# nv-tlabs/GEN3C

Hardware: NVIDIA H100
Metric: denoise-steps/sec, 7B DiT, 121-frame 720p latent (higher is better)
Workload: dtype bf16

## Files before the change

### gen3c_b200/_lib.py

```python
from __future__ import annotations

import ctypes as C
import os
from pathlib import Path

_HERE = Path(__file__).resolve().parent
LIB_PATH = _HERE / "lib" / "libgen3c_b200.so"


class G3CError(RuntimeError):
    pass


class DitConfig(C.Structure):
    _fields_ = [
        ("model_channels", C.c_int),
        ("num_blocks", C.c_int),
        ("num_heads", C.c_int),
        ("ffn_dim", C.c_int),
        ("context_dim", C.c_int),
        ("adaln_lora_dim", C.c_int),
        ("in_channels", C.c_int),
        ("out_channels", C.c_int),
        ("concat_padding_mask", C.c_int),
        ("max_frames", C.c_int),
        ("max_h", C.c_int),
        ("max_w", C.c_int),
        ("rope_h_ratio", C.c_float),
        ("rope_w_ratio", C.c_float),
        ("rope_t_ratio", C.c_float),
        ("base_fps", C.c_int),
    ]


class StepArgs(C.Structure):
    _fields_ = [
        ("xt", C.c_void_p),
        ("gt_latent", C.c_void_p),
        ("aug_noise", C.c_void_p),
        ("indicator", C.c_void_p),
        ("cond_mask", C.c_void_p),
        ("pose_cond", C.c_void_p),
        ("padding_mask", C.c_void_p),
        ("ctx_cond", C.c_void_p),
        ("ctx_uncond", C.c_void_p),
        ("sigma", C.c_float),
        ("sigma_next", C.c_float),
        ("sigma_data", C.c_float),
        ("sigma_aug", C.c_float),
        ("guidance", C.c_float),
        ("xt_next", C.c_void_p),
        ("cond_mask_uncond", C.c_void_p),
        ("net_output", C.c_void_p),
    ]


_P = C.c_void_p
_I = C.c_int
_F = C.c_float

SIGNATURES = {
    "g3c_last_error": (C.c_char_p, []),
    "g3c_version": (_I, []),
    "g3c_device_info": (_I, [C.POINTER(_I), C.POINTER(_I), C.POINTER(_I)]),
    "g3c_render_create": (_I, [_I, _I, _I, C.POINTER(_P)]),
    "g3c_render_destroy": (_I, [_P]),
    "g3c_render_set_deterministic": (_I, [_P, _I]),
    "g3c_forward_warp": (_I, [_P, _P, _P, _P, _P, _P, _I, _I, _I, _P, _P, _P, _P, _P]),
    "g3c_render_cache": (_I, [_P, _P, _P, _P, _P, _P, _I, _I, _I, _I, _I, _P, _P, _P, _P]),
    "g3c_bilinear_splatting": (_I, [_P, _P, _P, _P, _P, _I, _I, _I, _P, _P, _P]),
    "g3c_splat_indices": (_I, [_P, _I, _I, _I, _P, _P]),
    "g3c_unproject_points": (_I, [_P, _P, _P, _P, _I, _I, _I, _I, _P, _P]),
    "g3c_reliable_depth_mask": (_I, [_P, _I, _I, _I, _I, _F, _F, _P, _P]),
    "g3c_align_depth_nonrigid": (_I, [_P, _P, _P, _P, _P, _I, _I, _I, _F, _F, _P, _P]),
    "g3c_foreground_occlusion": (_I, [_P, _P, _P, _P, _I, _I, _I, _I, _P, _P, _P, _P]),
    "g3c_render_cache_occlusion": (_I, [_P, _P, _P, _P, _I, _I, _I, _I, _P, _P, _P, _I, _I, _P]),
    "g3c_gemm_bf16": (_I, [_P, _P, _P, _I, _I, _I, _I, _I, _I, _I, _P, _I, _P]),
    "g3c_gemm_norm_rope_bf16": (_I, [_P, _P, _P, _I, _I, _I, _I, _I, _I, _P, _P, _F, _P]),
    "g3c_attn_fwd": (_I, [_P, _P, _P, _P, _I, _I, _I, _I, _I, _I, _I, _F, _P]),
    "g3c_attn_fwd_sbhd": (_I, [_P, _P, _P, _P, _I, _I, _I, _I, _I, _I, _I, _I, _F, _P]),
    "g3c_attn_set_trace": (_I, [_P]),
    "g3c_ln_modulate": (_I, [_P, _P, _P, _P, _P, _I, _I, _F, _P]),
    "g3c_rmsnorm_rope": (_I, [_P, _I, _I, _I, _P, _P, _F, _P]),
    "g3c_dit_create": (_I, [C.POINTER(DitConfig), C.POINTER(_P)]),
    "g3c_dit_destroy": (_I, [_P]),
    "g3c_dit_load": (_I, [_P, C.c_char_p, _P, C.POINTER(C.c_int64), _I, _I]),
    "g3c_nccl_unique_id": (_I, [_P]),
    "g3c_dit_enable_cp": (_I, [_P, _P, _I, _I]),
    "g3c_dit_cp_export": (_I, [_P, _P]),
    "g3c_dit_cp_import": (_I, [_P, _P, _I]),
    "g3c_dit_cp_mode": (_I, [_P]),
    "g3c_dit_disable_cp": (_I, [_P]),
    "g3c_dit_enable_cfg_parallel": (_I, [_P, _I]),
    "g3c_dit_cfg_export": (_I, [_P, _P]),
    "g3c_dit_cfg_import": (_I, [_P, _P]),
    "g3c_dit_set_shape": (_I, [_P, _I, _I, _I, _I, _F]),
    "g3c_dit_forward": (_I, [_P, _P, _P, _P, _P, _F, _P, _P, _P]),
    "g3c_denoise_step": (_I, [_P, C.POINTER(StepArgs), _P]),
    "g3c_dit_profile": (_I, [_P, _I]),
    "g3c_dit_profile_read": (_I, [_P, C.POINTER(_F), C.POINTER(_I), _I]),
    "g3c_dit_profile_wait_ms": (_I, [_P, C.POINTER(_F)]),
    "g3c_dit_workspace_bytes": (C.c_int64, [_P]),
    "g3c_dit_last_launch_count": (_I, [_P]),
}

_lib = None


def load() -> C.CDLL:
    global _lib
    if _lib is not None:
        return _lib
    path = os.environ.get("GEN3C_B200_LIB", str(LIB_PATH))
    if not os.path.exists(path):
        raise G3CError(
            f"{path} not found: build it with `python -c 'import __graft_entry__ as g; g.build()'` "
            "(there is no CPU fallback)"
        )
    lib = C.CDLL(path)
    for name, (res, args) in SIGNATURES.items():
        fn = getattr(lib, name)
        fn.restype = res
        fn.argtypes = args
    _lib = lib
    return lib


def check(rc: int, what: str = "") -> None:
    if rc != 0:
        msg = load().g3c_last_error().decode("utf-8", "replace")
        raise G3CError(f"{what} failed with status {rc}: {msg}")


def ptr(t) -> int | None:
    if t is None:
        return None
    if not t.is_contiguous():
        raise G3CError("tensor passed to the C ABI must be contiguous")
    return t.data_ptr()


def stream_ptr() -> int:
    import torch

    return torch.cuda.current_stream().cuda_stream
```

### gen3c_b200/csrc/common.cuh

```cuda
#pragma once
#include <cuda.h>
#include <cuda_bf16.h>
#include <cuda_runtime.h>
#include <stdint.h>
#include <stdio.h>

#include "../../include/gen3c_b200.h"
#include "wgmma_ops.cuh"

namespace g3c {

void set_error(const char* fmt, ...);
int cuda_fail(cudaError_t e, const char* what, const char* file, int line);
#define G3C_CUDA(x)                                                         \
  do {                                                                      \
    cudaError_t _e = (x);                                                   \
    if (_e != cudaSuccess) return ::g3c::cuda_fail(_e, #x, __FILE__, __LINE__); \
  } while (0)
#define G3C_REQUIRE(cond, ...)        \
  do {                                \
    if (!(cond)) {                    \
      ::g3c::set_error(__VA_ARGS__);  \
      return G3C_EINVAL;       \
    }                                 \
  } while (0)

int make_tmap_bf16_sw128(CUtensorMap* out, const void* base, int rank, const uint64_t* dims,
                         const uint64_t* strides_bytes, const uint32_t* box);
int make_tmap_f32_sw128(CUtensorMap* out, const void* base, const uint64_t* dims,
                        const uint64_t* strides_bytes, const uint32_t* box);

int sm_count();

#ifdef __CUDACC__
__device__ __forceinline__ uint32_t smem_u32(const void* p) {
  return static_cast<uint32_t>(__cvta_generic_to_shared(p));
}
__device__ __forceinline__ uint32_t lane_id() { return threadIdx.x & 31; }
__device__ __forceinline__ uint32_t warp_id() { return __shfl_sync(0xffffffffu, threadIdx.x >> 5, 0); }

__device__ __forceinline__ bool elect_one() {
  uint32_t pred = 0;
  asm volatile(
      "{\n\t.reg .pred P;\n\t"
      "elect.sync _|P, 0xffffffff;\n\t"
      "selp.b32 %0, 1, 0, P;\n\t}\n"
      : "=r"(pred));
  return pred != 0;
}

__device__ __forceinline__ void mbar_init(uint64_t* bar, uint32_t count) {
  asm volatile("mbarrier.init.shared::cta.b64 [%0], %1;\n" ::"r"(smem_u32(bar)), "r"(count));
}
__device__ __forceinline__ void fence_barrier_init() {
  asm volatile("fence.mbarrier_init.release.cluster;\n" ::: "memory");
}
__device__ __forceinline__ void fence_proxy_async() {
  asm volatile("fence.proxy.async.shared::cta;\n" ::: "memory");
}
__device__ __forceinline__ void mbar_expect_tx(uint64_t* bar, uint32_t bytes) {
  asm volatile("mbarrier.arrive.expect_tx.shared::cta.b64 _, [%0], %1;\n" ::"r"(smem_u32(bar)),
               "r"(bytes)
               : "memory");
}
__device__ __forceinline__ void mbar_arrive(uint64_t* bar) {
  asm volatile("mbarrier.arrive.shared::cta.b64 _, [%0];\n" ::"r"(smem_u32(bar)) : "memory");
}
#ifndef G3C_MBAR_SUSPEND_NS
#define G3C_MBAR_SUSPEND_NS 0
#endif
__device__ __forceinline__ bool mbar_try_wait(uint64_t* bar, uint32_t parity) {
  uint32_t ok;
#if G3C_MBAR_SUSPEND_NS > 0
  asm volatile(
      "{\n\t.reg .pred P;\n\t"
      "mbarrier.try_wait.parity.shared::cta.b64 P, [%1], %2, %3;\n\t"
      "selp.b32 %0, 1, 0, P;\n\t}\n"
      : "=r"(ok)
      : "r"(smem_u32(bar)), "r"(parity), "r"((uint32_t)G3C_MBAR_SUSPEND_NS)
      : "memory");
#else
  asm volatile(
      "{\n\t.reg .pred P;\n\t"
      "mbarrier.try_wait.parity.shared::cta.b64 P, [%1], %2;\n\t"
      "selp.b32 %0, 1, 0, P;\n\t}\n"
      : "=r"(ok)
      : "r"(smem_u32(bar)), "r"(parity)
      : "memory");
#endif
  return ok != 0;
}
__device__ __forceinline__ bool mbar_test(uint64_t* bar, uint32_t parity) {
  uint32_t ok;
  asm volatile(
      "{\n\t.reg .pred P;\n\t"
      "mbarrier.test_wait.parity.shared::cta.b64 P, [%1], %2;\n\t"
      "selp.b32 %0, 1, 0, P;\n\t}\n"
      : "=r"(ok)
      : "r"(smem_u32(bar)), "r"(parity)
      : "memory");
  return ok != 0;
}
#ifndef G3C_MBAR_TIMEOUT_NS
#define G3C_MBAR_TIMEOUT_NS 4000000000ull
#endif
__device__ __forceinline__ uint64_t global_timer_ns() {
  uint64_t t;
  asm volatile("mov.u64 %0, %%globaltimer;\n" : "=l"(t));
  return t;
}
#ifdef G3C_MBAR_DEBUG
#define G3C_MBAR_TIMEOUT_ACTION(bar, parity)                                                                 \
  do {                                                                                                       \
    printf("g3c: mbarrier timeout block(%d,%d) thread %d bar@%u parity %u\n", blockIdx.x, blockIdx.y,        \
           threadIdx.x, bar, parity);                                                                        \
    __trap();                                                                                                \
  } while (0)
#else
#define G3C_MBAR_TIMEOUT_ACTION(bar, parity) asm volatile("trap;\n")
#endif
__device__ __forceinline__ void mbar_wait(uint64_t* bar, uint32_t parity) {
  if (mbar_try_wait(bar, parity)) return;
  uint32_t spins = 0;
  uint64_t t0 = 0;
  while (!mbar_try_wait(bar, parity)) {
    if ((++spins & 0xFFFu) == 0) {
      uint64_t now = global_timer_ns();
      if (t0 == 0) t0 = now;
      else if (now - t0 > G3C_MBAR_TIMEOUT_NS) G3C_MBAR_TIMEOUT_ACTION(smem_u32(bar), parity);
    }
  }
}

__device__ __forceinline__ void mbar_wait_ns(uint64_t* bar, uint32_t parity, unsigned long long timeout_ns) {
  if (mbar_try_wait(bar, parity)) return;
  uint32_t spins = 0;
  uint64_t t0 = 0;
  while (!mbar_try_wait(bar, parity)) {
    if ((++spins & 0xFFFu) == 0) {
      uint64_t now = global_timer_ns();
      if (t0 == 0) t0 = now;
      else if (now - t0 > timeout_ns) G3C_MBAR_TIMEOUT_ACTION(smem_u32(bar), parity);
    }
  }
}

__device__ __forceinline__ void mbar_wait_ns_or_exit(uint64_t* bar, uint32_t parity, unsigned long long timeout_ns) {
  if (mbar_try_wait(bar, parity)) return;
  uint32_t spins = 0;
  uint64_t t0 = 0;
  while (!mbar_try_wait(bar, parity)) {
    if ((++spins & 0xFFFu) == 0) {
      uint64_t now = global_timer_ns();
      if (t0 == 0) t0 = now;
      else if (now - t0 > timeout_ns) asm volatile("exit;\n");
    }
  }
}

__device__ __forceinline__ void tma_prefetch_desc(const CUtensorMap* m) {
  asm volatile("prefetch.tensormap [%0];\n" ::"l"(reinterpret_cast<uint64_t>(m)) : "memory");
}
__device__ __forceinline__ void tma_load_2d(void* smem_dst, const CUtensorMap* m, uint64_t* bar,
                                            int c0, int c1) {
  asm volatile(
      "cp.async.bulk.tensor.2d.shared::cluster.global.mbarrier::complete_tx::bytes"
      " [%0], [%1, {%3, %4}], [%2];\n" ::"r"(smem_u32(smem_dst)),
      "l"(reinterpret_cast<uint64_t>(m)), "r"(smem_u32(bar)), "r"(c0), "r"(c1)
      : "memory");
}
__device__ __forceinline__ void tma_load_3d(void* smem_dst, const CUtensorMap* m, uint64_t* bar,
                                            int c0, int c1, int c2) {
  asm volatile(
      "cp.async.bulk.tensor.3d.shared::cluster.global.mbarrier::complete_tx::bytes"
      " [%0], [%1, {%3, %4, %5}], [%2];\n" ::"r"(smem_u32(smem_dst)),
      "l"(reinterpret_cast<uint64_t>(m)), "r"(smem_u32(bar)), "r"(c0), "r"(c1), "r"(c2)
      : "memory");
}

__device__ __forceinline__ void tma_store_2d(const CUtensorMap* m, const void* smem_src, int c0, int c1) {
  asm volatile("cp.async.bulk.tensor.2d.global.shared::cta.bulk_group [%0, {%2, %3}], [%1];\n" ::"l"(
                   reinterpret_cast<uint64_t>(m)),
               "r"(smem_u32(smem_src)), "r"(c0), "r"(c1)
               : "memory");
}
__device__ __forceinline__ void tma_reduce_add_2d(const CUtensorMap* m, const void* smem_src, int c0, int c1) {
  asm volatile("cp.reduce.async.bulk.tensor.2d.global.shared::cta.add.bulk_group [%0, {%2, %3}], [%1];\n" ::"l"(
                   reinterpret_cast<uint64_t>(m)),
               "r"(smem_u32(smem_src)), "r"(c0), "r"(c1)
               : "memory");
}
__device__ __forceinline__ void tma_store_commit() { asm volatile("cp.async.bulk.commit_group;\n" ::: "memory"); }
template <int N>
__device__ __forceinline__ void tma_store_wait_read() {
  asm volatile("cp.async.bulk.wait_group.read %0;\n" ::"n"(N) : "memory");
}
template <int N>
__device__ __forceinline__ void tma_store_wait_all() {
  asm volatile("cp.async.bulk.wait_group %0;\n" ::"n"(N) : "memory");
}

__device__ __forceinline__ void wgmma_fence() { asm volatile("wgmma.fence.sync.aligned;\n" ::: "memory"); }
__device__ __forceinline__ void wgmma_commit() { asm volatile("wgmma.commit_group.sync.aligned;\n" ::: "memory"); }
template <int N>
__device__ __forceinline__ void wgmma_wait() {
  asm volatile("wgmma.wait_group.sync.aligned %0;\n" ::"n"(N) : "memory");
}
template <int N>
__device__ __forceinline__ void fence_regs(float (&r)[N]) {
#pragma unroll
  for (int i = 0; i < N; ++i) asm volatile("" : "+f"(r[i])::"memory");
}
template <int N>
__device__ __forceinline__ void fence_regs(uint32_t (&r)[N]) {
#pragma unroll
  for (int i = 0; i < N; ++i) asm volatile("" : "+r"(r[i])::"memory");
}

__device__ __forceinline__ uint64_t make_sdesc_sw128(uint32_t smem_addr) {
  uint64_t d = 0;
  d |= static_cast<uint64_t>((smem_addr & 0x3FFFFu) >> 4);
  d |= static_cast<uint64_t>(1) << 16;
  d |= static_cast<uint64_t>(1024u >> 4) << 32;
  d |= static_cast<uint64_t>(1) << 62;
  return d;
}
__device__ __forceinline__ uint64_t make_sdesc_sw128_mn(uint32_t smem_addr, uint32_t mn_block_bytes) {
  uint64_t d = 0;
  d |= static_cast<uint64_t>((smem_addr & 0x3FFFFu) >> 4);
  d |= static_cast<uint64_t>((mn_block_bytes >> 4) & 0x3FFFu) << 16;
  d |= static_cast<uint64_t>(1024u >> 4) << 32;
  d |= static_cast<uint64_t>(1) << 62;
  return d;
}
__device__ __forceinline__ uint64_t sdesc_advance(uint64_t d, uint32_t bytes) {
  return d + static_cast<uint64_t>(bytes >> 4);
}

template <int N>
__device__ __forceinline__ void setmaxnreg_dec() {
  asm volatile("setmaxnreg.dec.sync.aligned.u32 %0;\n" ::"n"(N));
}
template <int N>
__device__ __forceinline__ void setmaxnreg_inc() {
  asm volatile("setmaxnreg.inc.sync.aligned.u32 %0;\n" ::"n"(N));
}

__device__ __forceinline__ uint32_t pack_bf16x2(float lo, float hi) {
  __nv_bfloat162 v = __floats2bfloat162_rn(lo, hi);
  return *reinterpret_cast<uint32_t*>(&v);
}
__device__ __forceinline__ float warp_max(float v) {
#pragma unroll
  for (int o = 16; o > 0; o >>= 1) v = fmaxf(v, __shfl_xor_sync(0xffffffffu, v, o));
  return v;
}
__device__ __forceinline__ float warp_sum(float v) {
#pragma unroll
  for (int o = 16; o > 0; o >>= 1) v += __shfl_xor_sync(0xffffffffu, v, o);
  return v;
}
#endif

}
```

### gen3c_b200/csrc/gemm_wgmma.cu

```cuda
#include <cstdlib>
#include <cstring>

#include "kernels.h"

namespace g3c {

constexpr int BM = 128;
constexpr int BK = 64;
constexpr int WG_K = 16;
constexpr int GEMM_THREADS = 384;

struct GemmParams {
  int M, N, K;
  int ldd;
  void* D;
  const float* gate;
  int num_m_blk, num_n_blk, num_k_blk;
  int super_n;
  const float* nr_gamma;
  const float* nr_cs;
  float nr_eps;
};

constexpr int EPI_NORM_ROPE_BF16 = 4;

template <int BN>
struct GemmSmem {
  static constexpr int kABytes = BM * BK * 2;
  static constexpr int kBBytes = BN * BK * 2;
  static constexpr int kStageBytes = kABytes + kBBytes;
  static constexpr int kStages = (192 * 1024) / kStageBytes;
  static constexpr int kBarBytes = 256;
  static constexpr int kTotal = kStages * kStageBytes + kBarBytes + 1024;
};

__device__ __forceinline__ float gelu_erf(float x) {
  return 0.5f * x * (1.0f + erff(x * 0.70710678118654752440f));
}

__device__ __forceinline__ void tile_coords(const GemmParams& p, int tile, int& m_blk, int& n_blk) {
  int per_super = p.num_m_blk * p.super_n;
  int sc = tile / per_super;
  int rem = tile - sc * per_super;
  int n0 = sc * p.super_n;
  int width = p.num_n_blk - n0 < p.super_n ? p.num_n_blk - n0 : p.super_n;
  m_blk = rem / width;
  n_blk = n0 + rem - m_blk * width;
}

template <int BN>
__device__ __forceinline__ void epilogue_norm_rope(const float (&acc)[BN / 2], const GemmParams& p, int row_a, int col_q,
                                                   int n_base) {
#pragma unroll
  for (int hd = 0; hd < BN / 128; ++hd) {
    if (n_base + hd * 128 >= p.N) break;
    float ss[2] = {0.f, 0.f};
#pragma unroll
    for (int i = 16 * hd; i < 16 * hd + 16; ++i) {
      ss[0] = fmaf(acc[4 * i], acc[4 * i], fmaf(acc[4 * i + 1], acc[4 * i + 1], ss[0]));
      ss[1] = fmaf(acc[4 * i + 2], acc[4 * i + 2], fmaf(acc[4 * i + 3], acc[4 * i + 3], ss[1]));
    }
#pragma unroll
    for (int h = 0; h < 2; ++h) {
      ss[h] += __shfl_xor_sync(0xffffffffu, ss[h], 1);
      ss[h] += __shfl_xor_sync(0xffffffffu, ss[h], 2);
    }
#pragma unroll
    for (int h = 0; h < 2; ++h) {
      const int row = row_a + 8 * h;
      if (row >= p.M) continue;
      const float rstd = rsqrtf(ss[h] * (1.0f / 128.0f) + p.nr_eps);
      const float* cs = p.nr_cs ? p.nr_cs + (size_t)row * 128 : nullptr;
      __nv_bfloat16* dptr = reinterpret_cast<__nv_bfloat16*>(p.D) + (size_t)row * p.ldd + n_base + hd * 128;
#pragma unroll
      for (int i = 0; i < 8; ++i) {
        const int c = 8 * i + col_q;
        const float2 ga = *reinterpret_cast<const float2*>(p.nr_gamma + c);
        const float2 gb = *reinterpret_cast<const float2*>(p.nr_gamma + 64 + c);
        const int ia = 4 * (16 * hd + i) + 2 * h, ib = 4 * (16 * hd + i + 8) + 2 * h;
        float a[2] = {acc[ia] * (rstd * ga.x), acc[ia + 1] * (rstd * ga.y)};
        float b[2] = {acc[ib] * (rstd * gb.x), acc[ib + 1] * (rstd * gb.y)};
        if (cs) {
          const float2 co = *reinterpret_cast<const float2*>(cs + c);
          const float2 si = *reinterpret_cast<const float2*>(cs + 64 + c);
          const float cv[2] = {co.x, co.y}, sv[2] = {si.x, si.y};
#pragma unroll
          for (int e = 0; e < 2; ++e) {
            const float n = a[e] * cv[e] - b[e] * sv[e], m = b[e] * cv[e] + a[e] * sv[e];
            a[e] = n;
            b[e] = m;
          }
        }
        *reinterpret_cast<uint32_t*>(dptr + c) = pack_bf16x2(a[0], a[1]);
        *reinterpret_cast<uint32_t*>(dptr + 64 + c) = pack_bf16x2(b[0], b[1]);
      }
    }
  }
}

template <int BN, int EPI>
__device__ __forceinline__ void epilogue(const float (&acc)[BN / 2], const GemmParams& p, int row_a, int col_q,
                                         int n_base) {
  if constexpr (EPI == EPI_NORM_ROPE_BF16) {
    epilogue_norm_rope<BN>(acc, p, row_a, col_q, n_base);
  } else {
#pragma unroll
    for (int h = 0; h < 2; ++h) {
      const int row = row_a + 8 * h;
      if (row >= p.M) continue;
#pragma unroll
      for (int i = 0; i < BN / 8; ++i) {
        const int col = n_base + 8 * i + col_q;
        if (col >= p.N) continue;
        const bool pair = col + 1 < p.N;
        float v0 = acc[4 * i + 2 * h], v1 = acc[4 * i + 2 * h + 1];
        if constexpr (EPI == G3C_EPI_BF16 || EPI == G3C_EPI_GELU_BF16) {
          if constexpr (EPI == G3C_EPI_GELU_BF16) {
            v0 = gelu_erf(v0);
            v1 = gelu_erf(v1);
          }
          __nv_bfloat16* dptr = reinterpret_cast<__nv_bfloat16*>(p.D) + (size_t)row * p.ldd + col;
          if (pair) *reinterpret_cast<uint32_t*>(dptr) = pack_bf16x2(v0, v1);
          else dptr[0] = __float2bfloat16_rn(v0);
        } else {
          float* dptr = reinterpret_cast<float*>(p.D) + (size_t)row * p.ldd + col;
          if constexpr (EPI == G3C_EPI_GATED_RESIDUAL_F32) {
            if (pair) {
              const float2 g = *reinterpret_cast<const float2*>(p.gate + col);
              float2 x = *reinterpret_cast<float2*>(dptr);
              x.x = fmaf(g.x, v0, x.x);
              x.y = fmaf(g.y, v1, x.y);
              *reinterpret_cast<float2*>(dptr) = x;
            } else {
              dptr[0] = fmaf(p.gate[col], v0, dptr[0]);
            }
          } else {
            if (pair) *reinterpret_cast<float2*>(dptr) = make_float2(v0, v1);
            else dptr[0] = v0;
          }
        }
      }
    }
  }
}

template <int BN, int EPI>
__global__ void __launch_bounds__(GEMM_THREADS, 1)
    k_gemm(const __grid_constant__ CUtensorMap tmA, const __grid_constant__ CUtensorMap tmB, const GemmParams p) {
  using S = GemmSmem<BN>;
  constexpr int kStages = S::kStages;
  extern __shared__ uint8_t smem_raw[];
  uint8_t* smem = reinterpret_cast<uint8_t*>((reinterpret_cast<uintptr_t>(smem_raw) + 1023) &
                                             ~static_cast<uintptr_t>(1023));
  uint8_t* smem_a = smem;
  uint8_t* smem_b = smem + kStages * S::kABytes;
  uint64_t* bars = reinterpret_cast<uint64_t*>(smem + kStages * S::kStageBytes);
  uint64_t* full = bars;
  uint64_t* empty = bars + kStages;

  const uint32_t wg = threadIdx.x / 128;
  const uint32_t tid = threadIdx.x % 128;

  if (threadIdx.x == 0) {
    tma_prefetch_desc(&tmA);
    tma_prefetch_desc(&tmB);
    for (int i = 0; i < kStages; ++i) {
      mbar_init(&full[i], 1);
      mbar_init(&empty[i], 2);
    }
    fence_barrier_init();
  }
  __syncthreads();

  const int num_tiles = p.num_m_blk * p.num_n_blk;

  if (wg == 0) {
    setmaxnreg_dec<40>();
    if (tid == 0) {
      uint32_t stage = 0, phase = 0;
      for (int tile = blockIdx.x; tile < num_tiles; tile += gridDim.x) {
        int m_blk, n_blk;
        tile_coords(p, tile, m_blk, n_blk);
        for (int kb = 0; kb < p.num_k_blk; ++kb) {
          mbar_wait(&empty[stage], phase ^ 1);
          mbar_expect_tx(&full[stage], S::kStageBytes);
          tma_load_2d(smem_a + stage * S::kABytes, &tmA, &full[stage], kb * BK, m_blk * BM);
          tma_load_2d(smem_b + stage * S::kBBytes, &tmB, &full[stage], kb * BK, n_blk * BN);
          if (++stage == kStages) {
            stage = 0;
            phase ^= 1;
          }
        }
      }
    }
  } else {
    setmaxnreg_inc<232>();
    const uint32_t c = wg - 1;
    const uint32_t warp = tid / 32, lane = tid % 32;
    uint32_t stage = 0, phase = 0;
    float acc[BN / 2];
    for (int tile = blockIdx.x; tile < num_tiles; tile += gridDim.x) {
      int m_blk, n_blk;
      tile_coords(p, tile, m_blk, n_blk);
      uint32_t prev_stage = 0;
      for (int kb = 0; kb < p.num_k_blk; ++kb) {
        mbar_wait(&full[stage], phase);
        const uint64_t da = make_sdesc_sw128(smem_u32(smem_a + stage * S::kABytes + c * 64 * 128));
        const uint64_t db = make_sdesc_sw128(smem_u32(smem_b + stage * S::kBBytes));
        wgmma_fence();
#pragma unroll
        for (int k = 0; k < BK / WG_K; ++k) {
          const uint64_t a = sdesc_advance(da, k * WG_K * 2), b = sdesc_advance(db, k * WG_K * 2);
          const uint32_t accumulate = (kb | k) != 0 ? 1u : 0u;
          if constexpr (BN == 256) wgmma_ss_n256(acc, a, b, accumulate);
          else if constexpr (BN == 128) wgmma_ss_n128(acc, a, b, accumulate);
          else wgmma_ss_n64(acc, a, b, accumulate);
        }
        wgmma_commit();
        wgmma_wait<1>();
        fence_regs(acc);
        if (kb > 0 && tid == 0) mbar_arrive(&empty[prev_stage]);
        prev_stage = stage;
        if (++stage == kStages) {
          stage = 0;
          phase ^= 1;
        }
      }
      wgmma_wait<0>();
      fence_regs(acc);
      if (tid == 0) mbar_arrive(&empty[prev_stage]);
      epilogue<BN, EPI>(acc, p, m_blk * BM + (int)(c * 64 + warp * 16 + lane / 4), (int)(2 * (lane % 4)), n_blk * BN);
    }
  }
}

template <int BN, int EPI>
static int launch_gemm(const CUtensorMap& tmA, const CUtensorMap& tmB, const GemmParams& p, cudaStream_t st) {
  using S = GemmSmem<BN>;
  static bool configured = false;
  if (!configured) {
    G3C_CUDA(cudaFuncSetAttribute(k_gemm<BN, EPI>, cudaFuncAttributeMaxDynamicSharedMemorySize, S::kTotal));
    configured = true;
  }
  int tiles = p.num_m_blk * p.num_n_blk;
  int grid = tiles < sm_count() ? tiles : sm_count();
  k_gemm<BN, EPI><<<grid, GEMM_THREADS, S::kTotal, st>>>(tmA, tmB, p);
  G3C_CUDA(cudaGetLastError());
  return G3C_OK;
}

template <int BN>
static int dispatch_epi(int epi, const CUtensorMap& tmA, const CUtensorMap& tmB, const GemmParams& p, cudaStream_t st) {
  switch (epi) {
    case G3C_EPI_BF16: return launch_gemm<BN, G3C_EPI_BF16>(tmA, tmB, p, st);
    case G3C_EPI_GELU_BF16: return launch_gemm<BN, G3C_EPI_GELU_BF16>(tmA, tmB, p, st);
    case G3C_EPI_GATED_RESIDUAL_F32: return launch_gemm<BN, G3C_EPI_GATED_RESIDUAL_F32>(tmA, tmB, p, st);
    case G3C_EPI_F32: return launch_gemm<BN, G3C_EPI_F32>(tmA, tmB, p, st);
    case EPI_NORM_ROPE_BF16:
      if constexpr (BN >= 128) return launch_gemm<BN, EPI_NORM_ROPE_BF16>(tmA, tmB, p, st);
      break;
  }
  set_error("gemm: unknown epilogue %d", epi);
  return G3C_EINVAL;
}

int gemm_bf16(const void* A, const void* B, void* D, int M, int N, int K, int lda, int ldb, int ldd,
              int epilogue, const float* gate, int block_n, cudaStream_t st, const NormRope* norm_rope) {
  G3C_REQUIRE(A && B && D, "gemm: null operand");
  if (norm_rope) {
    G3C_REQUIRE(epilogue == G3C_EPI_BF16 && N % 128 == 0 && norm_rope->gamma,
                "gemm: the RMSNorm/RoPE epilogue needs the bf16 epilogue, N %% 128 == 0 and a gain vector");
    G3C_REQUIRE((reinterpret_cast<uintptr_t>(norm_rope->gamma) & 15) == 0 &&
                    (reinterpret_cast<uintptr_t>(norm_rope->cs) & 15) == 0,
                "gemm: RMSNorm gain / RoPE table must be 16-byte aligned");
    epilogue = EPI_NORM_ROPE_BF16;
  }
  G3C_REQUIRE(M > 0 && N > 0 && K > 0, "gemm: bad shape %dx%dx%d", M, N, K);
  G3C_REQUIRE(K % 8 == 0 && lda % 8 == 0 && ldb % 8 == 0, "gemm: K/lda/ldb must be multiples of 8");
  G3C_REQUIRE(lda >= K && ldb >= K && ldd >= N, "gemm: leading dimension smaller than extent");
  if (epilogue == G3C_EPI_BF16 || epilogue == G3C_EPI_GELU_BF16 || epilogue == EPI_NORM_ROPE_BF16)
    G3C_REQUIRE(ldd % 8 == 0 && (reinterpret_cast<uintptr_t>(D) & 15) == 0,
                "gemm: bf16 output needs ldd %% 8 == 0 and 16-byte aligned base");
  else
    G3C_REQUIRE(ldd % 4 == 0 && (reinterpret_cast<uintptr_t>(D) & 15) == 0,
                "gemm: f32 output needs ldd %% 4 == 0 and 16-byte aligned base");
  G3C_REQUIRE(epilogue != G3C_EPI_GATED_RESIDUAL_F32 ||
                  (gate && (reinterpret_cast<uintptr_t>(gate) & 15) == 0),
              "gemm: gated-residual epilogue needs a 16-byte aligned gate vector");
  int bn = block_n;
  G3C_REQUIRE(bn == 0 || bn == 64 || bn == 128 || bn == 256 || bn == 512, "gemm: block_n %d unsupported", bn);
  if (bn == 512) {
    G3C_REQUIRE(N % 256 == 0, "gemm: block_n 512 needs N %% 256 == 0 (N=%d)", N);
    bn = 256;
  }
  if (bn == 0) bn = (N >= 256 && N % 256 == 0) ? 256 : (N > 64 ? 128 : 64);
  G3C_REQUIRE(epilogue != EPI_NORM_ROPE_BF16 || bn >= 128, "gemm: the RMSNorm/RoPE epilogue needs tiles of whole heads");

  CUtensorMap tmA, tmB;
  uint64_t dimsA[2] = {(uint64_t)K, (uint64_t)M}, strA[1] = {(uint64_t)lda * 2};
  uint32_t boxA[2] = {BK, BM};
  int rc = make_tmap_bf16_sw128(&tmA, A, 2, dimsA, strA, boxA);
  if (rc) return rc;
  uint64_t dimsB[2] = {(uint64_t)K, (uint64_t)N}, strB[1] = {(uint64_t)ldb * 2};
  uint32_t boxB[2] = {BK, (uint32_t)bn};
  rc = make_tmap_bf16_sw128(&tmB, B, 2, dimsB, strB, boxB);
  if (rc) return rc;

  GemmParams p;
  p.M = M;
  p.N = N;
  p.K = K;
  p.ldd = ldd;
  p.D = D;
  p.gate = gate;
  p.nr_gamma = norm_rope ? norm_rope->gamma : nullptr;
  p.nr_cs = norm_rope ? norm_rope->cs : nullptr;
  p.nr_eps = norm_rope ? norm_rope->eps : 0.0f;
  p.num_m_blk = (M + BM - 1) / BM;
  p.num_n_blk = (N + bn - 1) / bn;
  p.num_k_blk = (K + BK - 1) / BK;
  long long col_bytes = (long long)bn * K * 2;
  int sn = (int)((16ll << 20) / (col_bytes > 0 ? col_bytes : 1));
  if (sn < 1) sn = 1;
  if (sn > p.num_n_blk) sn = p.num_n_blk;
  p.super_n = sn;
  switch (bn) {
    case 64: return dispatch_epi<64>(epilogue, tmA, tmB, p, st);
    case 128: return dispatch_epi<128>(epilogue, tmA, tmB, p, st);
    default: return dispatch_epi<256>(epilogue, tmA, tmB, p, st);
  }
}

}

extern "C" int g3c_gemm_bf16(const void* A, const void* B, void* D, int M, int N, int K, int lda,
                             int ldb, int ldd, int epilogue, const float* gate, int block_n,
                             void* stream) {
  return g3c::gemm_bf16(A, B, D, M, N, K, lda, ldb, ldd, epilogue, gate, block_n,
                        (cudaStream_t)stream);
}

extern "C" int g3c_gemm_norm_rope_bf16(const void* A, const void* B, void* D, int M, int N, int K, int lda, int ldb,
                                       int ldd, const float* gamma, const float* cos_sin, float eps, void* stream) {
  g3c::NormRope nr;
  nr.gamma = gamma;
  nr.cs = cos_sin;
  nr.eps = eps;
  return g3c::gemm_bf16(A, B, D, M, N, K, lda, ldb, ldd, G3C_EPI_BF16, nullptr, 0, (cudaStream_t)stream, &nr);
}
```

### gen3c_b200/ops.py

```python
from __future__ import annotations

from typing import Optional

import torch

from . import _lib

EPI_BF16, EPI_GELU_BF16, EPI_GATED_RESIDUAL_F32, EPI_F32 = 0, 1, 2, 3


def _chk(t: torch.Tensor, dtype, name: str):
    if not t.is_cuda or t.dtype != dtype or not t.is_contiguous():
        raise ValueError(f"{name} must be a contiguous CUDA tensor of dtype {dtype}")


def gemm(a: torch.Tensor, b: torch.Tensor, epilogue: int = EPI_BF16, out: Optional[torch.Tensor] = None,
         gate: Optional[torch.Tensor] = None, block_n: int = 0) -> torch.Tensor:
    _chk(a, torch.bfloat16, "a")
    _chk(b, torch.bfloat16, "b")
    M, K = a.shape
    N, K2 = b.shape
    assert K == K2, "inner dimensions differ"
    odt = torch.bfloat16 if epilogue in (EPI_BF16, EPI_GELU_BF16) else torch.float32
    if out is None:
        if epilogue == EPI_GATED_RESIDUAL_F32:
            raise ValueError("gated-residual epilogue accumulates into `out`")
        out = torch.empty((M, N), device=a.device, dtype=odt)
    _chk(out, odt, "out")
    if gate is not None:
        _chk(gate, torch.float32, "gate")
    lib = _lib.load()
    with torch.cuda.device(a.device):
        _lib.check(lib.g3c_gemm_bf16(_lib.ptr(a), _lib.ptr(b), _lib.ptr(out), M, N, K, K, K, N, epilogue,
                                     _lib.ptr(gate), block_n, _lib.stream_ptr()), "g3c_gemm_bf16")
    return out


def gemm_norm_rope(a: torch.Tensor, b: torch.Tensor, gamma: torch.Tensor, cos_sin: Optional[torch.Tensor] = None,
                   eps: float = 1e-6) -> torch.Tensor:
    _chk(a, torch.bfloat16, "a")
    _chk(b, torch.bfloat16, "b")
    _chk(gamma, torch.float32, "gamma")
    M, K = a.shape
    N = b.shape[0]
    assert b.shape[1] == K and N % 128 == 0 and gamma.numel() == 128
    if cos_sin is not None:
        _chk(cos_sin, torch.float32, "cos_sin")
        assert tuple(cos_sin.shape) == (M, 128)
    out = torch.empty((M, N), device=a.device, dtype=torch.bfloat16)
    lib = _lib.load()
    with torch.cuda.device(a.device):
        _lib.check(lib.g3c_gemm_norm_rope_bf16(_lib.ptr(a), _lib.ptr(b), _lib.ptr(out), M, N, K, K, K, N, _lib.ptr(gamma),
                                               _lib.ptr(cos_sin), eps, _lib.stream_ptr()), "g3c_gemm_norm_rope_bf16")
    return out


def attention(q: torch.Tensor, k: torch.Tensor, vt: torch.Tensor, heads: int, scale: Optional[float] = None,
              vt_chunk_len: int = 0) -> torch.Tensor:
    for t, n in ((q, "q"), (k, "k"), (vt, "vt")):
        _chk(t, torch.bfloat16, n)
    Lq, Dq = q.shape
    Lk = k.shape[0]
    assert Dq == heads * 128 and k.shape[1] == heads * 128
    o = torch.empty_like(q)
    if scale is None:
        scale = 128 ** -0.5
    lib = _lib.load()
    with torch.cuda.device(q.device):
        _lib.check(lib.g3c_attn_fwd(_lib.ptr(q), _lib.ptr(k), _lib.ptr(vt), _lib.ptr(o), Lq, Lk, heads, Dq, Dq, Dq,
                                    vt_chunk_len, scale, _lib.stream_ptr()), "g3c_attn_fwd")
    return o


def _token_stride(t: torch.Tensor, name: str) -> int:
    if not t.is_cuda or t.dtype != torch.bfloat16:
        raise ValueError(f"{name} must be a bf16 CUDA tensor, got {t.dtype} on {t.device}")
    if t.dim() != 4 or t.shape[0] < 1 or t[0].numel() == 0:
        raise ValueError(f"{name} must be a non-empty [s, b, h, d] tensor, got shape {tuple(t.shape)}")
    if not t[0].is_contiguous():
        raise ValueError(f"the (b, h, d) block of {name} must be contiguous, got strides {t.stride()}")
    row = t[0].numel()
    ld = t.stride(0) if t.shape[0] > 1 else row
    if ld < row or ld % 8 != 0:
        raise ValueError(f"the token stride of {name} ({ld}) must be a multiple of 8 and >= b*h*d = {row}")
    if t.data_ptr() % 16 != 0:
        raise ValueError(f"{name} must start on a 16-byte boundary")
    return ld


def attention_sbhd(q: torch.Tensor, k: torch.Tensor, v: torch.Tensor, scale: Optional[float] = None) -> torch.Tensor:
    if q.dim() == 4 and q.shape[-1] != 128:
        raise NotImplementedError(f"head_dim {q.shape[-1]}: only 128 is implemented")
    if q.dim() == 4 and k.dim() == 4 and k.shape[2] != q.shape[2]:
        raise NotImplementedError(f"{k.shape[2]} key heads for {q.shape[2]} query heads: GQA is not implemented")
    ldq, ldk, ldv = _token_stride(q, "q"), _token_stride(k, "k"), _token_stride(v, "v")
    if k.shape != v.shape or k.shape[1:] != q.shape[1:]:
        raise ValueError(f"q {tuple(q.shape)}, k {tuple(k.shape)} and v {tuple(v.shape)} must agree in (b, h, d) "
                         "and k, v in s")
    if not (q.device == k.device == v.device):
        raise ValueError("q, k and v must be on one device")
    sq, b, h, d = q.shape
    o = torch.empty((sq, b, h * d), device=q.device, dtype=torch.bfloat16)
    if scale is None:
        scale = 128 ** -0.5
    lib = _lib.load()
    with torch.cuda.device(q.device):
        _lib.check(lib.g3c_attn_fwd_sbhd(q.data_ptr(), k.data_ptr(), v.data_ptr(), o.data_ptr(), sq, k.shape[0], b, h,
                                         ldq, ldk, ldv, b * h * d, scale, _lib.stream_ptr()), "g3c_attn_fwd_sbhd")
    return o


def ln_modulate(x: torch.Tensor, shift: torch.Tensor, scale: torch.Tensor, pos: Optional[torch.Tensor] = None,
                eps: float = 1e-6) -> torch.Tensor:
    _chk(x, torch.float32, "x")
    L, D = x.shape
    y = torch.empty((L, D), device=x.device, dtype=torch.bfloat16)
    lib = _lib.load()
    with torch.cuda.device(x.device):
        _lib.check(lib.g3c_ln_modulate(_lib.ptr(x), _lib.ptr(pos), _lib.ptr(shift), _lib.ptr(scale), _lib.ptr(y), L, D,
                                       eps, _lib.stream_ptr()), "g3c_ln_modulate")
    return y


def rmsnorm_rope_(qk: torch.Tensor, heads: int, gamma: torch.Tensor, cos_sin: Optional[torch.Tensor] = None,
                  eps: float = 1e-6) -> torch.Tensor:
    _chk(qk, torch.bfloat16, "qk")
    _chk(gamma, torch.float32, "gamma")
    L, ld = qk.shape
    lib = _lib.load()
    with torch.cuda.device(qk.device):
        _lib.check(lib.g3c_rmsnorm_rope(_lib.ptr(qk), ld, L, heads, _lib.ptr(gamma), _lib.ptr(cos_sin), eps,
                                        _lib.stream_ptr()), "g3c_rmsnorm_rope")
    return qk
```

### include/gen3c_b200.h

```cpp
#ifndef GEN3C_B200_H_
#define GEN3C_B200_H_

#include <stdint.h>

#ifdef __cplusplus
extern "C" {
#endif

#define G3C_OK 0
#define G3C_EINVAL (-1)
#define G3C_ECUDA (-2)
#define G3C_ENOMEM (-3)
#define G3C_ESTATE (-4)
#define G3C_ENCCL (-5)

const char* g3c_last_error(void);
int g3c_version(void);
int g3c_device_info(int* sm_count, int* cc_major, int* cc_minor);


typedef struct g3c_render g3c_render_t;

int g3c_render_create(int H, int W, int max_items_per_pass, g3c_render_t** out);
int g3c_render_destroy(g3c_render_t* r);

int g3c_render_set_deterministic(g3c_render_t* r, int on);

#define G3C_WARP_RENDER_DEPTH 1
#define G3C_WARP_NOT_IMAGE 2

int g3c_forward_warp(g3c_render_t* r, const float* points, const float* image, const float* mask,
                     const float* w2c, const float* K, int b, int C, int flags, float* warped,
                     float* mask_out, float* depth_out, float* flow_out, void* stream);

int g3c_render_cache(g3c_render_t* r, const float* points, const float* images, const float* masks,
                     const float* w2cs, const float* Ks, int B, int F_target, int N, int src_frames,
                     int render_depth, float* pixels, float* masks_out, float* depth_out,
                     void* stream);

int g3c_bilinear_splatting(g3c_render_t* r, const float* frame, const float* mask,
                           const float* depth, const float* flow, int b, int C, int is_image,
                           float* out, float* mask_out, void* stream);

int g3c_splat_indices(const float* flow, int b, int H, int W, int32_t* idx, void* stream);

int g3c_unproject_points(const float* depth, const float* w2c, const float* K, const uint8_t* mask,
                         int b, int H, int W, int is_depth, float* points, void* stream);

int g3c_reliable_depth_mask(const float* depth, int b, int H, int W, int window, float ratio_thresh,
                            float eps, uint8_t* out, void* stream);

int g3c_align_depth_nonrigid(const float* depth, const float* target_depth, const uint8_t* target_mask, const float* K,
                             const float* c2w, int H, int W, int num_iters, float lambda_arap, float lr,
                             float* out_depth, void* stream);

int g3c_foreground_occlusion(const float* points, const unsigned char* boundary, const float* w2c, const float* K, int b,
                             int C, int H, int W, float* warped, float* mask, float* depth, void* stream);

int g3c_render_cache_occlusion(const float* points, const unsigned char* boundary, const float* w2cs, const float* Ks, int B,
                               int F_target, int N, int src_frames, float* pixels, float* masks, float* depth, int H, int W,
                               void* stream);


#define G3C_EPI_BF16 0
#define G3C_EPI_GELU_BF16 1
#define G3C_EPI_GATED_RESIDUAL_F32 2
#define G3C_EPI_F32 3

int g3c_gemm_bf16(const void* A, const void* B, void* D, int M, int N, int K, int lda, int ldb,
                  int ldd, int epilogue, const float* gate, int block_n, void* stream);

int g3c_gemm_norm_rope_bf16(const void* A, const void* B, void* D, int M, int N, int K, int lda, int ldb, int ldd,
                            const float* gamma, const float* cos_sin, float eps, void* stream);

int g3c_attn_fwd(const void* q, const void* k, const void* vt, void* o, int Lq, int Lk, int heads,
                 int ldq, int ldk, int ldo, int vt_chunk_len, float scale, void* stream);

int g3c_attn_fwd_sbhd(const void* q, const void* k, const void* v, void* o, int Lq, int Lk, int batch, int heads,
                      int ldq, int ldk, int ldv, int ldo, float scale, void* stream);

int g3c_attn_set_trace(unsigned long long* device_buffer);

int g3c_ln_modulate(float* x, const void* pos_bf16, const float* shift, const float* scale,
                    void* y_bf16, int L, int D, float eps, void* stream);

int g3c_rmsnorm_rope(void* qk_bf16, int ld, int L, int heads, const float* gamma,
                     const float* cos_sin, float eps, void* stream);

typedef struct g3c_dit g3c_dit_t;

typedef struct g3c_dit_config {
  int model_channels;
  int num_blocks;
  int num_heads;
  int ffn_dim;
  int context_dim;
  int adaln_lora_dim;
  int in_channels;
  int out_channels;
  int concat_padding_mask;
  int max_frames;
  int max_h, max_w;
  float rope_h_ratio, rope_w_ratio, rope_t_ratio;
  int base_fps;
} g3c_dit_config;

#define G3C_DTYPE_BF16 0
#define G3C_DTYPE_F32 1

int g3c_dit_create(const g3c_dit_config* cfg, g3c_dit_t** out);
int g3c_dit_destroy(g3c_dit_t* h);
int g3c_dit_load(g3c_dit_t* h, const char* name, const void* ptr, const int64_t* shape, int ndim,
                 int dtype);

int g3c_nccl_unique_id(void* out128);
int g3c_dit_enable_cp(g3c_dit_t* h, const void* nccl_unique_id, int cp_rank, int cp_size);
int g3c_dit_cp_export(g3c_dit_t* h, void* out_handle64);
int g3c_dit_cp_import(g3c_dit_t* h, const void* handles, int n);
int g3c_dit_cp_mode(const g3c_dit_t* h);
int g3c_dit_disable_cp(g3c_dit_t* h);

int g3c_dit_enable_cfg_parallel(g3c_dit_t* h, int role);
int g3c_dit_cfg_export(g3c_dit_t* h, void* out_handle64);
int g3c_dit_cfg_import(g3c_dit_t* h, const void* partner_handle64);

int g3c_dit_set_shape(g3c_dit_t* h, int T_local, int H_latent, int W_latent, int ctx_len, float fps);

int g3c_dit_forward(g3c_dit_t* h, const void* x, const void* cond_mask, const void* cond_pose,
                    const void* padding_mask, float timestep, const void* ctx, void* out,
                    void* stream);

typedef struct g3c_step_args {
  const void* xt;
  const void* gt_latent;
  const float* aug_noise;
  const float* indicator;
  const void* cond_mask;
  const void* pose_cond;
  const void* padding_mask;
  const void* ctx_cond;
  const void* ctx_uncond;
  float sigma, sigma_next, sigma_data, sigma_aug, guidance;
  void* xt_next;
  const void* cond_mask_uncond;
  void* net_output;
} g3c_step_args;

int g3c_denoise_step(g3c_dit_t* h, const g3c_step_args* a, void* stream);

int g3c_dit_profile_wait_ms(g3c_dit_t* h, float* ms);
#define G3C_PROFILE_CATEGORIES 6
int g3c_dit_profile(g3c_dit_t* h, int enable);
int g3c_dit_profile_read(g3c_dit_t* h, float* ms_by_category, int* launches_by_category, int ncat);

int64_t g3c_dit_workspace_bytes(const g3c_dit_t* h);
int g3c_dit_last_launch_count(const g3c_dit_t* h);

#ifdef __cplusplus
}
#endif
#endif
```

Measured before the change: 0.1310.

## Add 2-CTA cluster GEMM with TMA multicast of shared B tiles

Adds a paired-CTA variant of the persistent WGMMA GEMM. Two CTAs in a cluster compute adjacent M blocks and share the B (weight) tile: each CTA loads half of it and multicasts that half to both CTAs. Empty barriers now take arrivals from both CTAs, so a stage is only reused once both consumers are done. The paired path is chosen automatically for N%256 tiles when there are enough tiles to fill all clusters, cutting L2 traffic for B at the cost of cluster scheduling constraints and cross-CTA synchronisation.

```diff
diff --git a/gen3c_b200/_lib.py b/gen3c_b200/_lib.py
--- a/gen3c_b200/_lib.py
+++ b/gen3c_b200/_lib.py
@@ -76,7 +76,8 @@
     "g3c_foreground_occlusion": (_I, [_P, _P, _P, _P, _I, _I, _I, _I, _P, _P, _P, _P]),
     "g3c_render_cache_occlusion": (_I, [_P, _P, _P, _P, _I, _I, _I, _I, _P, _P, _P, _I, _I, _P]),
     "g3c_gemm_bf16": (_I, [_P, _P, _P, _I, _I, _I, _I, _I, _I, _I, _P, _I, _P]),
-    "g3c_gemm_norm_rope_bf16": (_I, [_P, _P, _P, _I, _I, _I, _I, _I, _I, _P, _P, _F, _P]),
+    "g3c_gemm_norm_rope_bf16": (_I, [_P, _P, _P, _I, _I, _I, _I, _I, _I, _P, _P, _F, _I, _P]),
+    "g3c_gemm_pair_clusters": (_I, [C.POINTER(_I)]),
     "g3c_attn_fwd": (_I, [_P, _P, _P, _P, _I, _I, _I, _I, _I, _I, _I, _F, _P]),
     "g3c_attn_fwd_sbhd": (_I, [_P, _P, _P, _P, _I, _I, _I, _I, _I, _I, _I, _I, _F, _P]),
     "g3c_attn_set_trace": (_I, [_P]),
diff --git a/gen3c_b200/csrc/common.cuh b/gen3c_b200/csrc/common.cuh
--- a/gen3c_b200/csrc/common.cuh
+++ b/gen3c_b200/csrc/common.cuh
@@ -66,6 +66,22 @@
 __device__ __forceinline__ void mbar_arrive(uint64_t* bar) {
   asm volatile("mbarrier.arrive.shared::cta.b64 _, [%0];\n" ::"r"(smem_u32(bar)) : "memory");
 }
+__device__ __forceinline__ uint32_t cluster_ctarank() {
+  uint32_t r;
+  asm volatile("mov.u32 %0, %%cluster_ctarank;\n" : "=r"(r));
+  return r;
+}
+__device__ __forceinline__ void cluster_sync() {
+  asm volatile("barrier.cluster.arrive.release;\n\tbarrier.cluster.wait.acquire;\n" ::: "memory");
+}
+__device__ __forceinline__ void mbar_arrive_cluster(uint64_t* bar, uint32_t cta) {
+  asm volatile(
+      "{\n\t.reg .b32 remote;\n\t"
+      "mapa.shared::cluster.u32 remote, %0, %1;\n\t"
+      "mbarrier.arrive.shared::cluster.b64 _, [remote];\n\t}\n" ::"r"(smem_u32(bar)),
+      "r"(cta)
+      : "memory");
+}
 #ifndef G3C_MBAR_SUSPEND_NS
 #define G3C_MBAR_SUSPEND_NS 0
 #endif
@@ -169,6 +185,14 @@
       "l"(reinterpret_cast<uint64_t>(m)), "r"(smem_u32(bar)), "r"(c0), "r"(c1)
       : "memory");
 }
+__device__ __forceinline__ void tma_load_2d_multicast(void* smem_dst, const CUtensorMap* m, uint64_t* bar, int c0,
+                                                      int c1, uint16_t cta_mask) {
+  asm volatile(
+      "cp.async.bulk.tensor.2d.shared::cluster.global.mbarrier::complete_tx::bytes.multicast::cluster"
+      " [%0], [%1, {%3, %4}], [%2], %5;\n" ::"r"(smem_u32(smem_dst)),
+      "l"(reinterpret_cast<uint64_t>(m)), "r"(smem_u32(bar)), "r"(c0), "r"(c1), "h"(cta_mask)
+      : "memory");
+}
 __device__ __forceinline__ void tma_load_3d(void* smem_dst, const CUtensorMap* m, uint64_t* bar,
                                             int c0, int c1, int c2) {
   asm volatile(
diff --git a/gen3c_b200/csrc/gemm_wgmma.cu b/gen3c_b200/csrc/gemm_wgmma.cu
--- a/gen3c_b200/csrc/gemm_wgmma.cu
+++ b/gen3c_b200/csrc/gemm_wgmma.cu
@@ -144,7 +144,7 @@
   }
 }
 
-template <int BN, int EPI>
+template <int BN, int EPI, bool PAIR>
 __global__ void __launch_bounds__(GEMM_THREADS, 1)
     k_gemm(const __grid_constant__ CUtensorMap tmA, const __grid_constant__ CUtensorMap tmB, const GemmParams p) {
   using S = GemmSmem<BN>;
@@ -160,17 +160,20 @@
 
   const uint32_t wg = threadIdx.x / 128;
   const uint32_t tid = threadIdx.x % 128;
+  constexpr int kCtas = PAIR ? 2 : 1;
+  const uint32_t rank = PAIR ? cluster_ctarank() : 0;
 
   if (threadIdx.x == 0) {
     tma_prefetch_desc(&tmA);
     tma_prefetch_desc(&tmB);
     for (int i = 0; i < kStages; ++i) {
       mbar_init(&full[i], 1);
-      mbar_init(&empty[i], 2);
+      mbar_init(&empty[i], 2 * kCtas);
     }
     fence_barrier_init();
   }
-  __syncthreads();
+  if constexpr (PAIR) cluster_sync();
+  else __syncthreads();
 
   const int num_tiles = p.num_m_blk * p.num_n_blk;
 
@@ -178,14 +181,19 @@
     setmaxnreg_dec<40>();
     if (tid == 0) {
       uint32_t stage = 0, phase = 0;
-      for (int tile = blockIdx.x; tile < num_tiles; tile += gridDim.x) {
+      for (int tile = blockIdx.x / kCtas; tile < num_tiles; tile += gridDim.x / kCtas) {
         int m_blk, n_blk;
         tile_coords(p, tile, m_blk, n_blk);
+        m_blk = m_blk * kCtas + rank;
         for (int kb = 0; kb < p.num_k_blk; ++kb) {
           mbar_wait(&empty[stage], phase ^ 1);
           mbar_expect_tx(&full[stage], S::kStageBytes);
           tma_load_2d(smem_a + stage * S::kABytes, &tmA, &full[stage], kb * BK, m_blk * BM);
-          tma_load_2d(smem_b + stage * S::kBBytes, &tmB, &full[stage], kb * BK, n_blk * BN);
+          if constexpr (PAIR)
+            tma_load_2d_multicast(smem_b + stage * S::kBBytes + rank * (S::kBBytes / 2), &tmB, &full[stage], kb * BK,
+                                  n_blk * BN + rank * (BN / 2), 0b11);
+          else
+            tma_load_2d(smem_b + stage * S::kBBytes, &tmB, &full[stage], kb * BK, n_blk * BN);
           if (++stage == kStages) {
             stage = 0;
             phase ^= 1;
@@ -199,9 +207,10 @@
     const uint32_t warp = tid / 32, lane = tid % 32;
     uint32_t stage = 0, phase = 0;
     float acc[BN / 2];
-    for (int tile = blockIdx.x; tile < num_tiles; tile += gridDim.x) {
+    for (int tile = blockIdx.x / kCtas; tile < num_tiles; tile += gridDim.x / kCtas) {
       int m_blk, n_blk;
       tile_coords(p, tile, m_blk, n_blk);
+      m_blk = m_blk * kCtas + rank;
       uint32_t prev_stage = 0;
       for (int kb = 0; kb < p.num_k_blk; ++kb) {
         mbar_wait(&full[stage], phase);
@@ -219,7 +228,10 @@
         wgmma_commit();
         wgmma_wait<1>();
         fence_regs(acc);
-        if (kb > 0 && tid == 0) mbar_arrive(&empty[prev_stage]);
+        if (kb > 0 && tid == 0) {
+          mbar_arrive(&empty[prev_stage]);
+          if constexpr (PAIR) mbar_arrive_cluster(&empty[prev_stage], rank ^ 1);
+        }
         prev_stage = stage;
         if (++stage == kStages) {
           stage = 0;
@@ -228,36 +240,78 @@
       }
       wgmma_wait<0>();
       fence_regs(acc);
-      if (tid == 0) mbar_arrive(&empty[prev_stage]);
+      if (tid == 0) {
+        mbar_arrive(&empty[prev_stage]);
+        if constexpr (PAIR) mbar_arrive_cluster(&empty[prev_stage], rank ^ 1);
+      }
       epilogue<BN, EPI>(acc, p, m_blk * BM + (int)(c * 64 + warp * 16 + lane / 4), (int)(2 * (lane % 4)), n_blk * BN);
     }
   }
-}
-
-template <int BN, int EPI>
+  if constexpr (PAIR) cluster_sync();
+}
+
+template <bool PAIR>
+static cudaLaunchConfig_t launch_config(int ctas, size_t smem, cudaStream_t st, cudaLaunchAttribute* attr) {
+  cudaLaunchConfig_t cfg = {};
+  cfg.gridDim = dim3(ctas);
+  cfg.blockDim = dim3(GEMM_THREADS);
+  cfg.dynamicSmemBytes = smem;
+  cfg.stream = st;
+  if (PAIR) {
+    attr->id = cudaLaunchAttributeClusterDimension;
+    attr->val.clusterDim.x = 2;
+    attr->val.clusterDim.y = 1;
+    attr->val.clusterDim.z = 1;
+    cfg.attrs = attr;
+    cfg.numAttrs = 1;
+  }
+  return cfg;
+}
+
+static int pair_clusters(int* out) {
+  static int n = 0;
+  if (n == 0) {
+    using S = GemmSmem<256>;
+    auto* kernel = k_gemm<256, G3C_EPI_BF16, true>;
+    G3C_CUDA(cudaFuncSetAttribute(kernel, cudaFuncAttributeMaxDynamicSharedMemorySize, S::kTotal));
+    cudaLaunchAttribute attr;
+    cudaLaunchConfig_t cfg = launch_config<true>(sm_count() / 2 * 2, S::kTotal, nullptr, &attr);
+    G3C_CUDA(cudaOccupancyMaxActiveClusters(&n, kernel, &cfg));
+    G3C_REQUIRE(n > 0, "gemm: the device cannot hold one cluster of the paired kernel");
+  }
+  *out = n;
+  return G3C_OK;
+}
+
+template <int BN, int EPI, bool PAIR>
 static int launch_gemm(const CUtensorMap& tmA, const CUtensorMap& tmB, const GemmParams& p, cudaStream_t st) {
   using S = GemmSmem<BN>;
   static bool configured = false;
   if (!configured) {
-    G3C_CUDA(cudaFuncSetAttribute(k_gemm<BN, EPI>, cudaFuncAttributeMaxDynamicSharedMemorySize, S::kTotal));
+    G3C_CUDA(cudaFuncSetAttribute(k_gemm<BN, EPI, PAIR>, cudaFuncAttributeMaxDynamicSharedMemorySize, S::kTotal));
     configured = true;
   }
   int tiles = p.num_m_blk * p.num_n_blk;
-  int grid = tiles < sm_count() ? tiles : sm_count();
-  k_gemm<BN, EPI><<<grid, GEMM_THREADS, S::kTotal, st>>>(tmA, tmB, p);
-  G3C_CUDA(cudaGetLastError());
+  int slots = sm_count();
+  if (PAIR) {
+    int rc = pair_clusters(&slots);
+    if (rc) return rc;
+  }
+  cudaLaunchAttribute attr;
+  cudaLaunchConfig_t cfg = launch_config<PAIR>((PAIR ? 2 : 1) * (tiles < slots ? tiles : slots), S::kTotal, st, &attr);
+  G3C_CUDA(cudaLaunchKernelEx(&cfg, k_gemm<BN, EPI, PAIR>, tmA, tmB, p));
   return G3C_OK;
 }
 
-template <int BN>
+template <int BN, bool PAIR = false>
 static int dispatch_epi(int epi, const CUtensorMap& tmA, const CUtensorMap& tmB, const GemmParams& p, cudaStream_t st) {
   switch (epi) {
-    case G3C_EPI_BF16: return launch_gemm<BN, G3C_EPI_BF16>(tmA, tmB, p, st);
-    case G3C_EPI_GELU_BF16: return launch_gemm<BN, G3C_EPI_GELU_BF16>(tmA, tmB, p, st);
-    case G3C_EPI_GATED_RESIDUAL_F32: return launch_gemm<BN, G3C_EPI_GATED_RESIDUAL_F32>(tmA, tmB, p, st);
-    case G3C_EPI_F32: return launch_gemm<BN, G3C_EPI_F32>(tmA, tmB, p, st);
+    case G3C_EPI_BF16: return launch_gemm<BN, G3C_EPI_BF16, PAIR>(tmA, tmB, p, st);
+    case G3C_EPI_GELU_BF16: return launch_gemm<BN, G3C_EPI_GELU_BF16, PAIR>(tmA, tmB, p, st);
+    case G3C_EPI_GATED_RESIDUAL_F32: return launch_gemm<BN, G3C_EPI_GATED_RESIDUAL_F32, PAIR>(tmA, tmB, p, st);
+    case G3C_EPI_F32: return launch_gemm<BN, G3C_EPI_F32, PAIR>(tmA, tmB, p, st);
     case EPI_NORM_ROPE_BF16:
-      if constexpr (BN >= 128) return launch_gemm<BN, EPI_NORM_ROPE_BF16>(tmA, tmB, p, st);
+      if constexpr (BN >= 128) return launch_gemm<BN, EPI_NORM_ROPE_BF16, PAIR>(tmA, tmB, p, st);
       break;
   }
   set_error("gemm: unknown epilogue %d", epi);
@@ -289,11 +343,21 @@
               "gemm: gated-residual epilogue needs a 16-byte aligned gate vector");
   int bn = block_n;
   G3C_REQUIRE(bn == 0 || bn == 64 || bn == 128 || bn == 256 || bn == 512, "gemm: block_n %d unsupported", bn);
-  if (bn == 512) {
+  bool pair = bn == 512;
+  const int m_pairs = (M + 2 * BM - 1) / (2 * BM);
+  if (pair) {
     G3C_REQUIRE(N % 256 == 0, "gemm: block_n 512 needs N %% 256 == 0 (N=%d)", N);
     bn = 256;
   }
-  if (bn == 0) bn = (N >= 256 && N % 256 == 0) ? 256 : (N > 64 ? 128 : 64);
+  if (bn == 0) {
+    bn = (N >= 256 && N % 256 == 0) ? 256 : (N > 64 ? 128 : 64);
+    if (bn == 256) {
+      int clusters = 0;
+      int rc = pair_clusters(&clusters);
+      if (rc) return rc;
+      pair = (long long)m_pairs * (N / 256) >= clusters;
+    }
+  }
   G3C_REQUIRE(epilogue != EPI_NORM_ROPE_BF16 || bn >= 128, "gemm: the RMSNorm/RoPE epilogue needs tiles of whole heads");
 
   CUtensorMap tmA, tmB;
@@ -302,7 +366,7 @@
   int rc = make_tmap_bf16_sw128(&tmA, A, 2, dimsA, strA, boxA);
   if (rc) return rc;
   uint64_t dimsB[2] = {(uint64_t)K, (uint64_t)N}, strB[1] = {(uint64_t)ldb * 2};
-  uint32_t boxB[2] = {BK, (uint32_t)bn};
+  uint32_t boxB[2] = {BK, (uint32_t)(pair ? bn / 2 : bn)};
   rc = make_tmap_bf16_sw128(&tmB, B, 2, dimsB, strB, boxB);
   if (rc) return rc;
 
@@ -316,7 +380,7 @@
   p.nr_gamma = norm_rope ? norm_rope->gamma : nullptr;
   p.nr_cs = norm_rope ? norm_rope->cs : nullptr;
   p.nr_eps = norm_rope ? norm_rope->eps : 0.0f;
-  p.num_m_blk = (M + BM - 1) / BM;
+  p.num_m_blk = pair ? m_pairs : (M + BM - 1) / BM;
   p.num_n_blk = (N + bn - 1) / bn;
   p.num_k_blk = (K + BK - 1) / BK;
   long long col_bytes = (long long)bn * K * 2;
@@ -327,10 +391,16 @@
   switch (bn) {
     case 64: return dispatch_epi<64>(epilogue, tmA, tmB, p, st);
     case 128: return dispatch_epi<128>(epilogue, tmA, tmB, p, st);
-    default: return dispatch_epi<256>(epilogue, tmA, tmB, p, st);
-  }
-}
-
+    default: return pair ? dispatch_epi<256, true>(epilogue, tmA, tmB, p, st)
+                         : dispatch_epi<256>(epilogue, tmA, tmB, p, st);
+  }
+}
+
+}
+
+extern "C" int g3c_gemm_pair_clusters(int* clusters) {
+  G3C_REQUIRE(clusters, "gemm_pair_clusters: null argument");
+  return g3c::pair_clusters(clusters);
 }
 
 extern "C" int g3c_gemm_bf16(const void* A, const void* B, void* D, int M, int N, int K, int lda,
@@ -341,10 +411,11 @@
 }
 
 extern "C" int g3c_gemm_norm_rope_bf16(const void* A, const void* B, void* D, int M, int N, int K, int lda, int ldb,
-                                       int ldd, const float* gamma, const float* cos_sin, float eps, void* stream) {
+                                       int ldd, const float* gamma, const float* cos_sin, float eps, int block_n,
+                                       void* stream) {
   g3c::NormRope nr;
   nr.gamma = gamma;
   nr.cs = cos_sin;
   nr.eps = eps;
-  return g3c::gemm_bf16(A, B, D, M, N, K, lda, ldb, ldd, G3C_EPI_BF16, nullptr, 0, (cudaStream_t)stream, &nr);
-}
+  return g3c::gemm_bf16(A, B, D, M, N, K, lda, ldb, ldd, G3C_EPI_BF16, nullptr, block_n, (cudaStream_t)stream, &nr);
+}
diff --git a/gen3c_b200/ops.py b/gen3c_b200/ops.py
--- a/gen3c_b200/ops.py
+++ b/gen3c_b200/ops.py
@@ -37,7 +37,7 @@
 
 
 def gemm_norm_rope(a: torch.Tensor, b: torch.Tensor, gamma: torch.Tensor, cos_sin: Optional[torch.Tensor] = None,
-                   eps: float = 1e-6) -> torch.Tensor:
+                   eps: float = 1e-6, block_n: int = 0) -> torch.Tensor:
     _chk(a, torch.bfloat16, "a")
     _chk(b, torch.bfloat16, "b")
     _chk(gamma, torch.float32, "gamma")
@@ -51,7 +51,8 @@
     lib = _lib.load()
     with torch.cuda.device(a.device):
         _lib.check(lib.g3c_gemm_norm_rope_bf16(_lib.ptr(a), _lib.ptr(b), _lib.ptr(out), M, N, K, K, K, N, _lib.ptr(gamma),
-                                               _lib.ptr(cos_sin), eps, _lib.stream_ptr()), "g3c_gemm_norm_rope_bf16")
+                                               _lib.ptr(cos_sin), eps, block_n, _lib.stream_ptr()),
+                   "g3c_gemm_norm_rope_bf16")
     return out
 
 
diff --git a/include/gen3c_b200.h b/include/gen3c_b200.h
--- a/include/gen3c_b200.h
+++ b/include/gen3c_b200.h
@@ -71,7 +71,9 @@
                   int ldd, int epilogue, const float* gate, int block_n, void* stream);
 
 int g3c_gemm_norm_rope_bf16(const void* A, const void* B, void* D, int M, int N, int K, int lda, int ldb, int ldd,
-                            const float* gamma, const float* cos_sin, float eps, void* stream);
+                            const float* gamma, const float* cos_sin, float eps, int block_n, void* stream);
+
+int g3c_gemm_pair_clusters(int* clusters);
 
 int g3c_attn_fwd(const void* q, const void* k, const void* vt, void* o, int Lq, int Lk, int heads,
                  int ldq, int ldk, int ldo, int vt_chunk_len, float scale, void* stream);
```

After: 0.1319, median of 6. Within noise of the previous version (+0.7%).
